# brown-ivl/manus

Measured on AMD Instinct MI355X. Metric: train iters/sec (fwd+bwd) 300k Gaussians @1080p, 8 views; PSNR parity, higher is better.
Workload: dtype f32

## Files before the change

include/manus_hip.h:

```cpp
#ifndef MANUS_HIP_H
#define MANUS_HIP_H

#include <stddef.h>
#include <stdint.h>

#ifdef __cplusplus
extern "C" {
#endif

#define MGR_VERSION 100
#define MGR_CAM_FLOATS 40
#define MGR_TILE 16
#define MGR_MAX_BONES 32

enum {
    MGR_OK = 0,
    MGR_EINVAL = -1,
    MGR_ENOMEM = -2,
    MGR_EHIP = -3,
    MGR_EOVERFLOW = -4,
    MGR_ECUT = -6,
    MGR_ETIER = -7
};

// ... 30 lines not shown
                       const float* xyz, const float* log_scale, const float* rot,
                       const float* opacity_logit, const float* f_dc, const float* f_rest,
                       const float* skin_w, const float* transforms, const int32_t* radii,
                       const float* out_color, const float* dL_dcolor, float grad2d_scale, float* d_xyz,
                       float* d_log_scale, float* d_rot, float* d_opacity_logit, float* d_f_dc,
                       float* d_f_rest, float* d_skin_w, float* stat_grad2d, float* stat_vis,
                       int32_t* stat_radii, void* workspace, size_t workspace_bytes,
                       int64_t pair_capacity, int debug, void* stream);



int mgr_views_active_list(void* workspace, int V, int N, int W, int H, int64_t pair_capacity, const uint32_t** list,
                          const uint32_t** count);

int mgr_views_backward_run_lists(int on);

int mgr_sh_to_half(int N, const float* f_rest, void* out_half, void* stream);

int mgr_raster_layout(int V, int N, int W, int H, int64_t pair_capacity, size_t* out, int n_out);
int mgr_raster_record_bytes(void);

int mgr_raster_set_cut_margin(float frac_entries, int min_entries, float depth_range_frac, float depth_rel, int interior_only);
int mgr_raster_set_cut_penalty(int forwards);
int mgr_raster_set_status_mirror(const void* workspace, void* host_words);
int mgr_raster_status_tiers_sync(const void* workspace, int64_t* num_pairs, int32_t* overflow, int32_t* tiers,
                                 void* stream);
int mgr_raster_status_sync(const void* workspace, int64_t* num_pairs, int32_t* overflow,
                           void* stream);

int mgr_raster_debug_binning_sync(const void* workspace, int V, int N, int W, int H,
// ... 150 lines not shown
```

manus_amd/_lib.py:

```python
import ctypes
import os

import weakref

import torch

_HERE = os.path.dirname(os.path.abspath(__file__))
_VARIANT = os.environ.get("MANUS_HIP_VARIANT", "")
LIB_PATH = os.path.join(_HERE, "libmanus_hip%s.so" % ("_" + _VARIANT if _VARIANT else ""))
_LIB = None

MGR_CAM_FLOATS = 40
MGR_MAX_BONES = 32

c_int, c_i64, c_f32, c_vp, c_sz = ctypes.c_int, ctypes.c_int64, ctypes.c_float, ctypes.c_void_p, ctypes.c_size_t

SIGNATURES = {
    "mgr_version": (c_int, []),
    "mgr_build_variant": (c_int, []),
    "mgr_raster_repair_max_tiles": (c_int, []),
    "mgr_last_error": (ctypes.c_char_p, []),
    "mgr_raster_workspace_bytes": (c_sz, [c_int, c_int, c_int, c_int, c_i64]),
    "mgr_raster_forward": (c_int, [c_int, c_int, c_int, c_int, c_vp, c_vp, c_vp, c_i64, c_vp, c_i64, c_vp,
                                   c_i64, c_vp, c_i64, c_vp, c_vp, c_vp, c_sz, c_i64, c_int, c_vp]),
# ... 9 lines not shown
    "mgr_raster_set_status_mirror": (c_int, [c_vp, c_vp]),
    "mgr_raster_set_cut_margin": (c_int, [c_f32, c_int, c_f32, c_f32, c_int]),
    "mgr_raster_set_cut_penalty": (c_int, [c_int]),
    "mgr_raster_status_tiers_sync": (c_int, [c_vp, ctypes.POINTER(c_i64), ctypes.POINTER(ctypes.c_int32),
                                             ctypes.POINTER(ctypes.c_int32), c_vp]),
    "mgr_debug_pair_alpha": (c_int, [c_int, c_vp, c_vp, c_vp, c_vp, c_vp, c_vp]),
    "mgr_raster_debug_binning_sync": (c_int, [c_vp, c_int, c_int, c_int, c_int, c_i64, c_int, c_vp, c_vp,
                                              c_i64, c_vp]),
    "mgr_skin_weights_fwd": (c_int, [c_int, c_vp, c_vp, c_int, c_int, c_int, c_int, c_int, c_vp, c_vp, c_vp,
                                     c_vp]),
    "mgr_skin_weights_bwd": (c_int, [c_int, c_vp, c_vp, c_int, c_int, c_int, c_int, c_int, c_vp, c_vp, c_vp,
                                     c_vp, c_int, c_vp]),
    "mgr_skin_weights_bwd_indexed": (c_int, [c_int, c_vp, c_vp, c_int, c_int, c_int, c_int, c_int, c_vp, c_vp, c_vp,
                                             c_vp, c_vp, c_vp, c_int, c_vp]),
    "mgr_views_backward_run_lists": (c_int, [c_int]),
    "mgr_views_active_list": (c_int, [c_vp, c_int, c_int, c_int, c_int, c_i64, ctypes.POINTER(c_vp), ctypes.POINTER(c_vp)]),
    "mgr_lbs_cov_fwd": (c_int, [c_int, c_int, c_int, c_vp, c_vp, c_vp, c_vp, c_vp, c_vp, c_vp, c_vp, c_vp]),
    "mgr_lbs_cov_bwd": (c_int, [c_int, c_int, c_int, c_vp, c_vp, c_vp, c_vp, c_vp, c_vp, c_vp, c_vp, c_vp,
                                c_vp, c_vp, c_vp, c_vp]),
    "mgr_lbs_cov_fwd_rows": (c_int, [c_int, c_int, c_int, c_vp, c_vp, c_vp, c_vp, c_vp, c_vp, c_vp, c_vp, c_int, c_vp]),
    "mgr_lbs_cov_bwd_rows": (c_int, [c_int, c_int, c_int, c_vp, c_vp, c_vp, c_vp, c_vp, c_vp, c_vp, c_vp, c_int, c_vp,
                                     c_vp, c_vp, c_vp, c_vp]),
    "mgr_sh_color_fwd_rows": (c_int, [c_int, c_int, c_vp, c_vp, c_i64, c_vp, c_i64, c_int, c_vp, c_vp, c_vp]),
    "mgr_sh_color_bwd_rows": (c_int, [c_int, c_int, c_vp, c_vp, c_i64, c_vp, c_i64, c_int, c_vp, c_vp, c_vp, c_vp, c_vp,
                                      c_vp]),
    "mgr_sh_color_fwd": (c_int, [c_int, c_int, c_vp, c_vp, c_i64, c_vp, c_i64, c_vp, c_vp, c_vp]),
    "mgr_sh_color_bwd": (c_int, [c_int, c_int, c_vp, c_vp, c_i64, c_vp, c_i64, c_vp, c_vp, c_vp, c_vp, c_vp,
                                 c_vp]),
    "mgr_pack_camera": (c_int, [c_f32, c_f32, c_vp, c_vp, c_vp, c_vp, c_vp]),
    "mgr_bone_transforms": (c_int, [c_int, c_int, c_vp, c_vp, c_vp, c_vp]),
# ... 172 lines not shown
```

manus_amd/csrc/mgr_common.h:

```cpp
#pragma once
#include <hip/hip_runtime.h>
#include <stdint.h>
#include <stdio.h>
#include <string.h>

#include "../../include/manus_hip.h"

#define MGR_WAVE 64

extern thread_local char g_mgr_err[512];

static inline int mgr_fail(int code, const char* fmt, const char* a = "", const char* b = "") {
    snprintf(g_mgr_err, sizeof(g_mgr_err), fmt, a, b);
    return code;
}

#define MGR_HIP(call)                                                                      \
    do {                                                                                   \
        hipError_t e_ = (call);                                                            \
        if (e_ != hipSuccess) return mgr_fail(MGR_EHIP, "%s: %s", #call, hipGetErrorString(e_)); \
    } while (0)

#define MGR_LAUNCH_CHECK(name, stream, debug)                                              \
    do {                                                                                   \
// ... 106 lines not shown
    int32_t pad;
#if MGR_GREC_BYTES == 64
    int32_t pad64[4];
#endif
};

#define MGR_CHUNK 64

static inline uint32_t mgr_rep_units(int64_t cap) { int64_t u = cap / 16384; return (uint32_t)(u < 64 ? 64 : (u > 1024 ? 1024 : u)); }
static inline uint32_t mgr_rep_list(int64_t cap) { int64_t n = cap / 8; return (uint32_t)(n < (1 << 16) ? (1 << 16) : (n > (2 << 20) ? (2 << 20) : n)); }
static inline uint32_t mgr_rep_ck(int64_t cap) { return mgr_rep_list(cap) / MGR_CHUNK + mgr_rep_units(cap); }

struct MgrLayout {
    size_t header, scan_part, scan_cls, scan_box, grec, depth, rect, alive, pair_off, tile_count, tile_start, tile_cursor, tile_done, tile_qdone,
        tile_zcut, tile_zused, tile_qend, tile_bgok, tile_queue, tile_qrec, chunk_start, items, ckpt, keys, keys2, groups, sorted_gid, final_T, n_contrib, pair_tag, pair_grad, inst_grad, inst_tag,
        db_count, db_cursor, db_start, db_nvis, db_bbox, db_keys, db_order, db_rec, bin_mat, tile_rep, rep_unit, rep_state, rep_last, rep_cnt, rep_cand, rep_view, tile_zwin, db_zrange, db_item, total;
};

#ifndef MGR_DB_BUCKETS
#define MGR_DB_BUCKETS 1024
#endif
#ifndef MGR_DB_ITEM
#define MGR_DB_ITEM 768
#endif
#define MGR_DB_RANK_MAX 2048
#define MGR_DB_RANK_LARGE 3072
#ifndef MGR_BIN_BLOCK
#define MGR_BIN_BLOCK 1024
#endif
static inline int mgr_bin_block(int V, int N) { return (long long)V * (long long)N >= 500000ll ? MGR_BIN_BLOCK : 256; }

static inline size_t mgr_align(size_t x) { return (x + 255) & ~(size_t)255; }

static inline MgrLayout mgr_layout(int V, int N, int W, int H, int64_t cap) {
    MgrLayout L;
    size_t VN = (size_t)V * (size_t)(N > 0 ? N : 1);
    size_t gx = (W + MGR_TILE - 1) / MGR_TILE, gy = (H + MGR_TILE - 1) / MGR_TILE;
    size_t VT = (size_t)V * gx * gy, VP = (size_t)V * W * H;
    size_t c = (size_t)(cap > 0 ? cap : 1);
    size_t o = 0;
    L.header = o;      o += mgr_align(sizeof(MgrHeader));
    const size_t scan_blocks = (size_t)V * ((gx * gy + 1023) / 1024);
    L.scan_part = o;   o += mgr_align((scan_blocks + 1) * 8);
    L.scan_cls = o;    o += mgr_align(scan_blocks * 34 * 4);
    L.scan_box = o;    o += mgr_align(scan_blocks * 16);
    L.grec = o;        o += mgr_align(VN * sizeof(MgrGRec));
    L.depth = o;       o += mgr_align(VN * 4);
    L.rect = o;        o += mgr_align(VN * 8);
// ... 34 lines not shown
        L.db_order = o;  o += mgr_align(VN * 4);
        L.db_rec = o;    o += mgr_align(VN * 16);
        L.bin_mat = o;   o += mgr_align((size_t)V * nblk * gx * gy * 4);
    }
    L.tile_bgok = o; o += mgr_align((size_t)V * gx * gy);
    L.tile_rep = o;  o += mgr_align(VT * 4);
    L.rep_unit = o;  o += mgr_align(rep_u * sizeof(MgrRepUnit));
    L.rep_state = o; o += mgr_align(rep_u * 64 * 16);
    L.rep_last = o;  o += mgr_align(rep_u * 64 * 4);
    L.rep_cnt = o;   o += mgr_align(rep_u * 4);
    L.rep_cand = o;  o += mgr_align(rep_u * (size_t)MGR_REP_CAND * 8);
    L.rep_view = o;  o += mgr_align((size_t)V * sizeof(MgrRepView));
    L.tile_zwin = o; o += mgr_align(VT * 4);
    L.db_zrange = o; o += mgr_align((size_t)V * (((size_t)(N > 0 ? N : 1) + 511) / 512) * 2 * 4);
    L.db_item = o;   o += mgr_align((size_t)V * (((size_t)(N > 0 ? N : 1) + MGR_DB_ITEM - 1) / MGR_DB_ITEM + 1) * 2 * 4);
    L.total = o;
    return L;
}

#ifdef __HIPCC__

struct MgrCam {
    float tanfovx, tanfovy;
    float view[16], proj[16];
    float campos[3];
};

__device__ __forceinline__ void mgr_load_cam(const float* __restrict__ cams, int v, MgrCam& c) {
    const float* p = cams + (size_t)v * MGR_CAM_FLOATS;
    c.tanfovx = p[0];
    c.tanfovy = p[1];
#pragma unroll
    for (int i = 0; i < 16; ++i) {
        c.view[i] = p[2 + i];
// ... 305 lines not shown
```

manus_amd/csrc/raster_bwd.hip:

```cpp
#include <atomic>

#include "instance_math.h"

#ifdef MGR_STATS
__device__ unsigned long long g_stats[16];
extern "C" int mgr_debug_stats(unsigned long long* dst) {
    return (int)hipMemcpyFromSymbol(dst, HIP_SYMBOL(g_stats), sizeof(unsigned long long) * 16);
}
__device__ unsigned long long g_bhist[3][65];
extern "C" int mgr_debug_bhist(unsigned long long* dst) {
    return (int)hipMemcpyFromSymbol(dst, HIP_SYMBOL(g_bhist), sizeof(unsigned long long) * 3 * 65);
}
#define BH(r, c, v) do { const int c_ = (c); const unsigned long long v_ = (unsigned long long)(v); if (lane == 0) atomicAdd(&g_bhist[r][c_], v_); } while (0)
#define MGR_STAT(i, v) do { const unsigned long long v_ = (unsigned long long)(v); if (lane == 0) atomicAdd(&g_stats[i], v_); } while (0)
#else
#define MGR_STAT(i, v)
#endif

#ifdef BWD_PROF
__device__ unsigned long long g_bprof[8];
extern "C" int mgr_debug_bprof(unsigned long long* dst) {
    return (int)hipMemcpyFromSymbol(dst, HIP_SYMBOL(g_bprof), sizeof(unsigned long long) * 8);
}
#define BP(k) { const long long now_ = wall_clock64(); acc_[k] += now_ - tp_; tp_ = now_; }
// ... 26 lines not shown
    return bits;
}
#define MGR_LDS_VOLATILE_F32 volatile const __attribute__((address_space(3))) float*
#define BWD_ROW 288
#define BWD_PLANE_W 64
#define BWD_PLANE_B 128
#ifndef BWD_WAVES
#define BWD_WAVES 4
#endif

__global__ __launch_bounds__(256) __attribute__((amdgpu_waves_per_eu(BWD_WAVES, BWD_WAVES))) void k_blend_bwd(
    int N, int W, int H, int gx, int gy, const uint32_t* __restrict__ sorted_gid, const MgrGRec* __restrict__ grec,
    const uint32_t* __restrict__ n_contrib, const float4* __restrict__ ckpt, const uint4* __restrict__ items,
    MgrHeader* hdr, const float* __restrict__ out_color, const float* __restrict__ dL_dpix,
    uint32_t* __restrict__ pair_tag, float4* __restrict__ pair_grad, uint32_t* __restrict__ inst_tag, uint32_t cap,
    uint32_t epoch) {
    __shared__ __align__(16) float s_pair[4][32][MGR_PAIR_FLOATS];
    __shared__ __align__(16) float s_xch[4][4 * BWD_ROW];
    __shared__ float s_acc[4][BWD_BATCH][9];
    __shared__ uint32_t s_flag[4][BWD_BATCH];

    const int tid = threadIdx.x, wave = tid >> 6, lane = tid & 63;
    const int T = gx * gy;
    const uint32_t n_items = hdr->n_items;
    if (blockIdx.x == 0 && tid < 4) (tid == 3 ? hdr->n_active : hdr->n_runs[tid]) = 0;
    if (blockIdx.x == 0 && tid == 4) hdr->bwd_seq += 1u;
    const size_t P = (size_t)W * H;
    const unsigned long long lt = (1ull << lane) - 1ull;
    float* const slab = &s_pair[wave][0][0];
    float* const xch = &s_xch[wave][0];
    float* const acc = &s_acc[wave][0][0];
    uint32_t* const flag = &s_flag[wave][0];
    const int e2 = lane >> 3, pc = lane & 7;
#ifdef BWD_PROF
    long long acc_[6] = {0, 0, 0, 0, 0, 0}, tp_ = wall_clock64(), nit_ = 0;
#endif

    MgrQueue queue;
    queue.init(hdr->qctr, n_items, (int)blockIdx.x);
    uint32_t item = queue.resolve(queue.issue(lane), lane);
    while (item != 0xFFFFFFFFu) {
        const uint32_t next_raw = queue.issue(lane);
        const uint4 recA = items[2 * (size_t)item], recB = items[2 * (size_t)item + 1];
        const uint32_t vt = recA.x, chunk = recA.y;
        const uint32_t mxq[4] = {recB.x, recB.y, recB.z, recB.w};
        const int v = (int)(vt / (uint32_t)T), t = (int)(vt % (uint32_t)T);
        const int bx = t % gx, by = t / gx;
        const uint32_t first = chunk * BWD_BATCH;
        const uint32_t tmax = max(max(mxq[0], mxq[1]), max(mxq[2], mxq[3]));
        const int cnt = (int)min((uint32_t)BWD_BATCH, tmax - first);
        const MgrGRec* const gv = grec + (size_t)v * N;
#ifdef BWD_PROF
        ++nit_;
#endif
        BP(0);
#if BWD_KO & 1024
        const uint32_t gid = sorted_gid[recA.z] + 0u * (uint32_t)lane;
#else
        const uint32_t gid = sorted_gid[recA.z + (uint32_t)min(lane, cnt - 1)];
// ... 1 lines not shown
        float4 ra, rb, rcz;
        {
            const MgrGRec* r = gv + gid;
            ra = *(const float4*)r;
            rb = *((const float4*)r + 1);
            rcz = *((const float4*)r + 2);
        }
#pragma unroll
        for (int k = 0; k < 9; ++k) acc[k * 64 + lane] = 0.f;
        flag[lane] = 0u;
        const int32_t slot = __float_as_int(rcz.y) + by * __float_as_int(rcz.z) + bx;
        const float qmax_e = mgr_qmax(rb.y);
        BP(1);

        uint32_t qmask = (mxq[0] > first ? 1u : 0u) | (mxq[1] > first ? 2u : 0u) | (mxq[2] > first ? 4u : 0u) | (mxq[3] > first ? 8u : 0u);
        struct PxState {
            uint32_t nc;
            float t0, t1, t2, o0, o1, o2;
            float4 ck;
        };
        auto load_px = [&](int quad, PxState& q) {
            const int px = bx * 16 + (quad & 1) * 8 + (lane & 7);
            const int py = by * 16 + (quad >> 1) * 8 + (lane >> 3);
            const size_t pixc = (size_t)min(py, H - 1) * W + min(px, W - 1);
#if BWD_KO & 512
            q.nc = tmax; q.t0 = 0.001f * (float)pixc; q.t1 = 0.5f; q.t2 = 0.25f; q.o0 = 0.3f; q.o1 = 0.2f; q.o2 = 0.1f;
            q.ck = make_float4(0.1f, 0.1f, 0.1f, 0.5f);
#else
            q.nc = n_contrib[(size_t)v * P + pixc];
            const float* gp = dL_dpix + (size_t)v * 3 * P + pixc;
// ... 44 lines not shown
                xch[xoff] = g0; xch[64 + xoff] = g1; xch[128 + xoff] = g2;
                __builtin_amdgcn_wave_barrier();
#pragma unroll
                for (int j = 0; j < 2; ++j) {
                    const float4 a4 = *(const float4*)(xch + 4 * pc + 32 * j), b4 = *(const float4*)(xch + 64 + 4 * pc + 32 * j),
                                 c4 = *(const float4*)(xch + 128 + 4 * pc + 32 * j);
                    gr0[2 * j] = mgr_v2f{a4.x, a4.y}; gr0[2 * j + 1] = mgr_v2f{a4.z, a4.w};
                    gr1[2 * j] = mgr_v2f{b4.x, b4.y}; gr1[2 * j + 1] = mgr_v2f{b4.z, b4.w};
                    gr2[2 * j] = mgr_v2f{c4.x, c4.y}; gr2[2 * j + 1] = mgr_v2f{c4.z, c4.w};
                }
                __builtin_amdgcn_wave_barrier();
            }
            const float fx_col = qx0 + (float)pc;
            const mgr_v2f g0v = {g0, g0}, g1v = {g1, g1}, g2v = {g2, g2};
            bool alive = false;
            if (lane < cnt && first + (uint32_t)lane < wlast)
                alive = !mgr_box_dead(ra.x, ra.y, ra.z, ra.w, rb.x, qmax_e, qx0 + (float)bx0, qy0 + (float)by0,
                                      qx0 + (float)bx1, qy0 + (float)by1);
            const unsigned long long m = __ballot(alive);
            const int na = __popcll(m);
            MGR_STAT(0, __popcll(__ballot(lane < cnt)));
            MGR_STAT(1, na);
            if (alive) {
                const int rank = __popcll(m & lt);
                float* pb = slab + (rank >> 1) * MGR_PAIR_FLOATS;
                mgr_pair_store(pb, rank & 1, ra.x, ra.y, ra.z, ra.w, rb.x, rb.y, rb.z, rb.w, rcz.x,
                               first + (uint32_t)lane + 1u);
                if ((na & 1) && rank == na - 1) mgr_pair_pad(pb);
            }
            const int npair = (BWD_KO & 4) ? ((na + 1) >> 1) * 57 / 100 : (na + 1) >> 1;
#ifdef MGR_STATS
            MGR_STAT(8, (unsigned long long)npair * __popcll(__ballot(last > first)));
            MGR_STAT(9, npair);
// ... 767 lines not shown
    }
    const int b8 = (n8 + IB_THREADS / 8 - 1) / (IB_THREADS / 8), b4 = (n4 + IB_THREADS / 4 - 1) / (IB_THREADS / 4);
    if constexpr (NVV >= 8) {
        if (blk < b8) { inst_bwd_body<8, BMAX, MIXED, SH_HALF, true, NVV>(blk, n8, active_list, MGR_IB_ARGS); return; }
    }
    blk -= b8;
    if constexpr (NVV >= 4) {
        if (blk < b4) { inst_bwd_body<4, BMAX, MIXED, SH_HALF, true, NVV>(blk, n4, active_list + (size_t)N, MGR_IB_ARGS); return; }
    }
    blk -= b4;
    inst_bwd_body<2, BMAX, MIXED, SH_HALF, true, NVV>(blk, n2, active_list + 2 * (size_t)N, MGR_IB_ARGS);
}

static std::atomic<int> g_inst_runs{[] { const char* e = getenv("MANUS_INST_RUNS"); return e ? atoi(e) : 1; }()};
extern "C" int mgr_views_backward_run_lists(int on) { return g_inst_runs.exchange(on); }

struct CanonGrads {
    int B, n_art, sh_half;
    const float *xyz, *log_scale, *rot, *op_logit, *f_dc, *f_rest, *skin_w, *transforms;
    const int32_t* radii;
    float grad2d_scale;
    float *d_xyz, *d_ls, *d_rot, *d_op, *d_fdc, *d_frest, *d_w, *st_grad2d, *st_vis;
    int32_t* st_radii;
};

static int raster_backward_impl(int V, int N, int W, int H, const float* cams, const float* bg,
                                   const float* means3D, int64_t s_means, const float* cov3D,
                                   int64_t s_cov, const float* colors, int64_t s_col,
                                   const float* opacity, int64_t s_op, const float* out_color,
                                   const float* dL_dcolor, float* dL_dmeans3D, float* dL_dmeans2D, float* dL_dcolors,
// ... 9 lines not shown
    if (!canon && (!means3D || !cov3D || !dL_dmeans3D || !dL_dmeans2D || !dL_dcolors || !dL_dopacity || !dL_dcov3D))
        return mgr_fail(MGR_EINVAL, "mgr_raster_backward: null pointer");
    const int gx = (W + 15) / 16, gy = (H + 15) / 16;
    const MgrLayout L = mgr_layout(V, N, W, H, cap);
    if (workspace_bytes < L.total) return mgr_fail(MGR_ENOMEM, "mgr_raster_backward: workspace too small");
    char* ws = (char*)workspace;
    MgrHeader* hdr = (MgrHeader*)(ws + L.header);
    static std::atomic<uint32_t> g_epoch{0};
    uint32_t epoch = g_epoch.fetch_add(1) + 1;
    if (epoch == 0) epoch = g_epoch.fetch_add(1) + 1;

    { MGR_PROF("k_blend_bwd", stream); hipLaunchKernelGGL(k_blend_bwd, dim3(256 * BWD_WAVES), dim3(256), 0, stream, N, W, H, gx, gy,
                       (const uint32_t*)(ws + L.sorted_gid), (const MgrGRec*)(ws + L.grec), (const uint32_t*)(ws + L.n_contrib),
                       (const float4*)(ws + L.ckpt), (const uint4*)(ws + L.items), hdr, out_color,
                       dL_dcolor, (uint32_t*)(ws + L.pair_tag), (float4*)(ws + L.pair_grad),
                       (uint32_t*)(ws + L.inst_tag), (uint32_t)cap, epoch); }
    MGR_LAUNCH_CHECK("k_blend_bwd", stream, debug & 1);
    if (canon) {
        const int Gv = V <= 1 ? 1 : V <= 2 ? 2 : V <= 4 ? 4 : 8;
        const int ipb = 256 / Gv;
        const size_t lds = (size_t)Gv * (MGR_CAM_FLOATS + (canon->skin_w ? IB_TSTRIDE(canon->B) : 0)) * sizeof(float);
        float4* iacc = (float4*)(ws + L.inst_grad);
        uint32_t* alist = (uint32_t*)(ws + L.inst_grad + (size_t)N * Gv * 48);
        const int ipb2 = IB_THREADS / Gv;
        const bool mixed = canon->skin_w && canon->n_art < N;
        int rounds = (int)((long long)N / ((long long)ipb * 1024));
        rounds = rounds < 1 ? 1 : (rounds > IG_ROUNDS ? IG_ROUNDS : rounds);
        const dim3 grid((N + ipb2 - 1) / ipb2), grid_g((N + ipb * rounds - 1) / (ipb * rounds));
        for (int v0 = 0; v0 < V; v0 += Gv) {
            const int vc = V - v0 < Gv ? V - v0 : Gv;
            const int accm = v0 > 0 ? 1 : 0;
// ... 138 lines not shown
```

manus_amd/csrc/raster_fwd.hip:

```cpp
#include <atomic>
#include <mutex>

#include "instance_math.h"
#include "il_list.h"

#include <cstdlib>
#include <cstring>
#include <map>
#include <string>
#include <vector>

thread_local char g_mgr_err[512] = {0};

int g_mgr_prof_on = 0;
namespace {
struct ProfRec { const char* name; hipEvent_t a, b; };
std::vector<ProfRec> g_prof_recs;
std::vector<hipEvent_t> g_prof_pool;
hipEvent_t prof_event() {
    if (!g_prof_pool.empty()) { hipEvent_t e = g_prof_pool.back(); g_prof_pool.pop_back(); return e; }
    hipEvent_t e;
    if (hipEventCreate(&e) != hipSuccess) return nullptr;
    return e;
}
// ... 1838 lines not shown
    return (int)e;
}
#endif
__device__ __forceinline__ float mgr_sel(unsigned long long m, float a, float b) {
    float r;
    asm("v_cndmask_b32 %0, %1, %2, %3" : "=v"(r) : "v"(b), "v"(a), "s"(m));
    return r;
}
__device__ __forceinline__ uint32_t mgr_selu(unsigned long long m, uint32_t a, uint32_t b) {
    uint32_t r;
    asm("v_cndmask_b32 %0, %1, %2, %3" : "=v"(r) : "v"(b), "v"(a), "s"(m));
    return r;
}
__device__ __forceinline__ bool mgr_fwd_pair_step(const float4& R0, const float4& R1, const float4& R2, const float4& R3, const float4& R4,
                                                  const mgr_v2f fpx2, const mgr_v2f fpy2, float& Tr, mgr_v2f& C01, float& C2, uint32_t& last,
                                                  unsigned long long& done_m, const unsigned long long exec_m) {
    mgr_v2f al;
    unsigned long long ma, mb;
    mgr_pair_alpha_masks(R0, R1, R2, fpx2, fpy2, al, ma, mb);
    {
        const unsigned long long keep = ma & ~done_m;
        const float a = mgr_sel(keep, al.x, 0.0f);
        const float testT = Tr * (1.0f - a);
        const unsigned long long stop = __builtin_amdgcn_ballot_w64(testT < 0.0001f);
        const unsigned long long contrib = keep & ~stop;
        const float w = mgr_sel(contrib, a * Tr, 0.0f);
        C01 += mgr_v2f{R3.x, R3.y} * w;
        C2 += R4.x * w;
        Tr = mgr_sel(stop, Tr, testT);
        last = mgr_selu(contrib, __float_as_uint(R4.z), last);
        done_m |= stop;
    }
    {
        const unsigned long long keep = mb & ~done_m;
        const float a = mgr_sel(keep, al.y, 0.0f);
        const float testT = Tr * (1.0f - a);
        const unsigned long long stop = __builtin_amdgcn_ballot_w64(testT < 0.0001f);
        const unsigned long long contrib = keep & ~stop;
        const float w = mgr_sel(contrib, a * Tr, 0.0f);
        C01 += mgr_v2f{R3.z, R3.w} * w;
        C2 += R4.y * w;
        Tr = mgr_sel(stop, Tr, testT);
        last = mgr_selu(contrib, __float_as_uint(R4.w), last);
        done_m |= stop;
    }
    return (~done_m & exec_m) == 0ull;
}
#define FWD_SLOTS 64
__global__ __launch_bounds__(256) FWD_OCC void k_blend_fwd(int N, int W, int H, int gx, int gy, int VT,
                                                     const float* __restrict__ bg,
                                                     const uint32_t* __restrict__ tile_queue,
                                                     const uint4* __restrict__ tile_qrec,
                                                     const uint32_t* __restrict__ sorted_gid,
                                                     const MgrGRec* __restrict__ grec,
                                                     float* __restrict__ out_color,
                                                     uint32_t* __restrict__ n_contrib,
                                                     uint32_t* __restrict__ tile_done,
                                                     uint32_t* __restrict__ tile_qdone,
                                                     float4* __restrict__ ckpt, MgrHeader* hdr,
                                                     const uint32_t* __restrict__ tile_zused, uint32_t* __restrict__ tile_qend, int skip_fill) {
    __shared__ __align__(16) float s_pair[4][32][MGR_PAIR_FLOATS];
    __shared__ __align__(16) uint4 s_qrec[FWD_SLOTS];
    __shared__ uint32_t s_step[FWD_SLOTS];
    __shared__ uint32_t s_claim;
    const int tid = threadIdx.x, lane = tid & 63;
    const int wave = __builtin_amdgcn_readfirstlane(tid >> 6);
    const int T = gx * gy;
    const uint32_t n_busy = hdr->queue_len;
    const uint32_t n_queue = hdr->queue_len_i;
    const size_t P = (size_t)W * H;
    const float bg0 = bg[0], bg1 = bg[1], bg2 = bg[2];
    const unsigned long long lt = (1ull << lane) - 1ull;
    float* const slab = &s_pair[wave][0][0];
    const uint32_t gid_max = (uint32_t)(N > 0 ? N - 1 : 0);

// ... 166 lines not shown
                const uint32_t nxt = queue.resolve(raw, lane);
                uint4 nrec = make_uint4(END, 0u, 0u, 0u);
                if (nxt != END) nrec = tile_qrec[nxt];
#ifdef FWD_KO_DEEP
                if (nxt != END && nxt < FWD_KO_DEEP) nrec.x = MGR_HOLE;
#endif
                if (lane == 0) {
                    s_qrec[(step + 1u) % FWD_SLOTS] = nrec;
                    __builtin_amdgcn_fence(__ATOMIC_RELEASE, "workgroup");
                    __hip_atomic_store(&s_step[(step + 1u) % FWD_SLOTS], step + 1u, __ATOMIC_RELAXED, __HIP_MEMORY_SCOPE_WORKGROUP);
                }
                provided = true;
            }
            const int npair = (cnt + 1) >> 1;
            FP(1);
            auto pair_step = [&](const float4& R0, const float4& R1, const float4& R2, const float4& R3, const float4& R4) -> bool {
                return mgr_fwd_pair_step(R0, R1, R2, R3, R4, fpx2, fpy2, Tr, C01, C2, last, done_m, exec_m);
            };
#ifdef FWD_LDS_PIPE1
            for (int p = 0; p < npair; ++p) {
                const float4* pp = (const float4*)(slab + p * MGR_PAIR_FLOATS);
                const float4 R0 = pp[0], R1 = pp[1], R2 = pp[2], R3 = pp[3], R4 = pp[4];
                if (pair_step(R0, R1, R2, R3, R4)) break;
            }
#else
            if (npair > 0) {
                const float4* pa = (const float4*)slab;
                float4 A0 = pa[0], A1 = pa[1], A2 = pa[2];
                for (int p = 0;; p += 2) {
                    const float4* pb = (const float4*)(slab + min(p + 1, 31) * MGR_PAIR_FLOATS);
                    const float4 B0 = pb[0], B1 = pb[1], B2 = pb[2];
                    const float4* pc = (const float4*)(slab + p * MGR_PAIR_FLOATS);
                    const float4 A3 = pc[3], A4 = pc[4];
                    __builtin_amdgcn_sched_barrier(0);
                    if (pair_step(A0, A1, A2, A3, A4) || p + 1 >= npair) break;
                    const float4* pn = (const float4*)(slab + min(p + 2, 31) * MGR_PAIR_FLOATS);
                    A0 = pn[0]; A1 = pn[1]; A2 = pn[2];
                    const float4 B3 = pb[3], B4 = pb[4];
                    __builtin_amdgcn_sched_barrier(0);
                    if (pair_step(B0, B1, B2, B3, B4) || p + 2 >= npair) break;
                }
            }
#endif
            FP(2);
            const uint32_t nextpos = off + 64u;
            if ((nextpos % MGR_CHUNK) == 0 && nextpos < nlist && (((~done_m & exec_m) >> lane) & 1ull))
                ckpt[(size_t)(ck0 + nextpos / MGR_CHUNK - 1) * 256 + pslot] = make_float4(C01.x, C01.y, C2, Tr);
#ifndef FWD_PF1
            rec = rec1;
            rec1 = rec2;
#endif
            FP(3);
        }
        FP(3);
        if (!provided) {
            const uint32_t nxt = queue.resolve(raw, lane);
            uint4 nrec = make_uint4(END, 0u, 0u, 0u);
            if (nxt != END) nrec = tile_qrec[nxt];
#ifdef FWD_KO_DEEP
            if (nxt != END && nxt < FWD_KO_DEEP) nrec.x = MGR_HOLE;
#endif
            if (lane == 0) {
// ... 296 lines not shown
                                      qy0 + (float)by1);
            }
            const unsigned long long m = __ballot(alive);
            const int cnt = __popcll(m);
            if (alive) {
                const int rank = __popcll(m & lt);
                float* pb = slab + (rank >> 1) * MGR_PAIR_FLOATS;
                mgr_pair_store<true>(pb, rank & 1, r.x, r.y, r.ca, r.cb, r.cc, r.op, r.r, r.g, r.b, nl + j + (uint32_t)lane + 1u);
                if ((cnt & 1) && rank == cnt - 1) mgr_pair_pad<true>(pb);
            }
            __builtin_amdgcn_wave_barrier();
            const int npair = (cnt + 1) >> 1;
            for (int p = 0; p < npair; ++p) {
                const float4* pp = (const float4*)(slab + p * MGR_PAIR_FLOATS);
                const float4 R0 = pp[0], R1 = pp[1], R2 = pp[2], R3 = pp[3], R4 = pp[4];
                if (mgr_fwd_pair_step(R0, R1, R2, R3, R4, fpx2, fpy2, Tr, C01, C2, last, done_m, exec_m)) break;
            }
            __builtin_amdgcn_wave_barrier();
            const uint32_t nextpos = nl + j + blen;
            if ((nextpos % MGR_CHUNK) == 0u && nextpos < total && (((~done_m & exec_m) >> lane) & 1ull))
                ckpt[(size_t)(ov_ck0 + nextpos / MGR_CHUNK - c0) * 256 + pslot] = make_float4(C01.x, C01.y, C2, Tr);
            j += blen;
        }
        if (inside) {
            const size_t pix = (size_t)py * W + px;
            n_contrib[(size_t)v * P + pix] = last;
            float* o = out_color + (size_t)v * 3 * P + pix;
            o[0] = C01.x + Tr * bg0;
            o[P] = C01.y + Tr * bg1;
            o[2 * P] = C2 + Tr * bg2;
        }
// ... 124 lines not shown
    const uint32_t base = s_base;
    for (uint32_t i = (uint32_t)tid; i < total; i += 256u) {
        int lo = 0, hi = 256;
        while (hi - lo > 1) {
            const int mid = (lo + hi) >> 1;
            if (s_run[mid] <= i) lo = mid; else hi = mid;
        }
        const uint32_t c = i - s_run[lo];
        const uint4 r = s_qr[lo], x = s_rp[lo];
        uint32_t off = r.y + c * MGR_CHUNK, ck = r.w + (c > 0 ? c - 1 : 0);
        const uint32_t p0 = x.x & 0x7FFFFFFFu;
        if (x.x != 0u && c * MGR_CHUNK >= p0) {
            off = x.y + (c * MGR_CHUNK - p0);
            ck = c * MGR_CHUNK == p0 ? x.w : x.z + (c - p0 / MGR_CHUNK);
        }
        items[2 * (size_t)(base + i)] = make_uint4(r.x, c, off, ck);
        items[2 * (size_t)(base + i) + 1] = s_qd[lo];
    }
}

struct CanonInputs {
    int B, n_art, sh_half;
    const float *xyz, *log_scale, *rot, *op_logit, *f_dc, *f_rest, *skin_w, *transforms;
};

struct MgrSideStream {
    hipStream_t stream = nullptr;
    hipEvent_t fork = nullptr, join = nullptr;
    hipError_t init() {
        if (stream) return hipSuccess;
        hipError_t e = hipStreamCreateWithFlags(&stream, hipStreamNonBlocking);
// ... 268 lines not shown
                           (const unsigned long long*)(ws + L.keys), (uint32_t*)(ws + L.sorted_gid), hdr,
                           (uint32_t)cap); }
        MGR_HIP(hipEventRecord(side.join, side.stream));
        { MGR_PROF("k_tile_sort", stream); hipLaunchKernelGGL(k_tile_sort, dim3(512), dim3(RS_THREADS), SORT_LDS_KEYS * 8 + RS_WAVES * 256 * 4 + 256, stream,
                           tile_start, (const uint32_t*)(ws + L.tile_queue),
                           (const unsigned long long*)(ws + L.keys), (const unsigned long long*)(ws + L.keys2),
                           (const uint4*)(ws + L.groups), (uint32_t*)(ws + L.sorted_gid), hdr, (uint32_t)cap); }
        MGR_HIP(hipStreamWaitEvent(stream, side.join, 0));
        MGR_LAUNCH_CHECK("k_tile_sort", stream, debug);
    }
    }
    if (!do_blend) return MGR_OK;
    { MGR_PROF("k_blend_fwd", stream); hipLaunchKernelGGL(k_blend_fwd, dim3(MGR_FWD_GRID), dim3(256), 0, stream, N, W, H, gx, gy, VT, bg,
                       (const uint32_t*)(ws + L.tile_queue), (const uint4*)(ws + L.tile_qrec), (const uint32_t*)(ws + L.sorted_gid), (const MgrGRec*)(ws + L.grec), out_color,
                       (uint32_t*)(ws + L.n_contrib), (uint32_t*)(ws + L.tile_done), (uint32_t*)(ws + L.tile_qdone),
                       (float4*)(ws + L.ckpt), hdr, (const uint32_t*)(ws + L.tile_zused), (uint32_t*)(ws + L.tile_qend), bg_filled ? 1 : 0); }
    if (repair && N > 0) {
        { MGR_PROF("k_repair_scan", stream);
          hipLaunchKernelGGL(k_repair_prep, dim3(V), dim3(256), 0, stream, T, gx, hdr, rep_all, (const uint32_t*)(ws + L.tile_zused),
                             (const uint32_t*)(ws + L.tile_zwin));
          hipLaunchKernelGGL(k_repair_scan, dim3(REP_SCAN_SEGS, V), dim3(REP_SCAN_THREADS), 0, stream, N, T, gx, hdr, rep_all, (const int32_t*)radii,
                             (const ushort4*)(ws + L.rect), (const float*)(ws + L.depth), (const MgrGRec*)(ws + L.grec)); }
        { MGR_PROF("k_repair_blend", stream);
          hipLaunchKernelGGL(k_repair_blend, dim3(128), dim3(RS_THREADS), REP_BLEND_LDS, stream, N, W, H, gx, T, hdr, rep_all, bg,
                             (uint32_t*)(ws + L.sorted_gid), (const MgrGRec*)(ws + L.grec), out_color, (uint32_t*)(ws + L.n_contrib),
                             (uint32_t*)(ws + L.tile_qdone), (float4*)(ws + L.ckpt)); }
        MGR_LAUNCH_CHECK("k_repair_blend", stream, debug);
    }
    IlListArgs ll = mgr_take_loss_list(workspace);
    if (ll.nbx) {
        if (ll.H != H || ll.W != W || ll.list_views != V) return mgr_fail(MGR_EINVAL, "attached loss list: views or image size differ from the forward's");
// ... 36 lines not shown
    return raster_forward_impl(V, N, W, H, cams, bg, nullptr, 0, nullptr, 0, nullptr, 0, nullptr, 0, &ci, out_color,
                               radii, workspace, workspace_bytes, cap, debug, stream_);
}

#ifdef BIN_PROF
extern "C" int mgr_binprof(unsigned long long* out) {
    MGR_HIP(hipMemcpyFromSymbol(out, HIP_SYMBOL(g_binprof), 8 * 8 * 4096));
    return 0;
}
#endif
extern "C" int mgr_raster_layout(int V, int N, int W, int H, int64_t cap, size_t* out, int n_out) {
    const MgrLayout L = mgr_layout(V, N, W, H, cap);
    const size_t v[] = {L.header, L.grec, L.depth, L.rect, L.alive, L.pair_off, L.tile_count, L.tile_start,
                        L.tile_cursor, L.tile_done, L.tile_queue, L.chunk_start, L.items, L.ckpt, L.keys,
                        L.sorted_gid, L.final_T, L.n_contrib, L.pair_tag, L.pair_grad, L.total, L.inst_grad, L.inst_tag,
                        L.db_nvis, L.db_bbox, L.db_order, L.tile_zcut, L.tile_zused, L.tile_qend, L.tile_rep, L.rep_unit, L.rep_cnt, L.tile_zwin};
    const int n = (int)(sizeof(v) / sizeof(v[0]));
    for (int i = 0; i < n && i < n_out; ++i) out[i] = v[i];
    return n;
}

__global__ void k_debug_pair_alpha(int n, const float* __restrict__ rec, const int32_t* __restrict__ px,
                                   const int32_t* __restrict__ py, float* __restrict__ alpha, int32_t* __restrict__ valid) {
    const int i = blockIdx.x * blockDim.x + threadIdx.x;
    if (i >= n) return;
    float pb[MGR_PAIR_FLOATS];
    const float* r = rec + (size_t)i * 6;
    mgr_pair_store(pb, 0, r[0], r[1], r[2], r[3], r[4], r[5], 0.f, 0.f, 0.f, 1u);
    mgr_pair_pad(pb);
    const float4 R0 = make_float4(pb[0], pb[1], pb[2], pb[3]), R1 = make_float4(pb[4], pb[5], pb[6], pb[7]),
                 R2 = make_float4(pb[8], pb[9], pb[10], pb[11]);
// ... 80 lines not shown
```

Baseline: 771.4.

## Record per-chunk contributor masks in forward blend and reuse them in backward

The forward blend kernel now records, for each 64-entry chunk and pixel quad, a ballot mask of the Gaussians that actually contributed. The backward blend reads these masks instead of re-running the conservative box-dead test, and drops quads with no contributors. This cuts wasted per-Gaussian work in the backward pass, at the cost of an extra workspace buffer and extra forward stores. Items from repair/other paths are flagged with the top bit of the chunk field so they fall back to the box test.

```diff
diff --git a/include/manus_hip.h b/include/manus_hip.h
--- a/include/manus_hip.h
+++ b/include/manus_hip.h
@@ -68,6 +68,8 @@
                           const uint32_t** count);
 
 int mgr_views_backward_run_lists(int on);
+
+int mgr_raster_bwd_boxtest(int on);
 
 int mgr_sh_to_half(int N, const float* f_rest, void* out_half, void* stream);
 
diff --git a/manus_amd/_lib.py b/manus_amd/_lib.py
--- a/manus_amd/_lib.py
+++ b/manus_amd/_lib.py
@@ -47,6 +47,7 @@
     "mgr_skin_weights_bwd_indexed": (c_int, [c_int, c_vp, c_vp, c_int, c_int, c_int, c_int, c_int, c_vp, c_vp, c_vp,
                                              c_vp, c_vp, c_vp, c_int, c_vp]),
     "mgr_views_backward_run_lists": (c_int, [c_int]),
+    "mgr_raster_bwd_boxtest": (c_int, [c_int]),
     "mgr_views_active_list": (c_int, [c_vp, c_int, c_int, c_int, c_int, c_i64, ctypes.POINTER(c_vp), ctypes.POINTER(c_vp)]),
     "mgr_lbs_cov_fwd": (c_int, [c_int, c_int, c_int, c_vp, c_vp, c_vp, c_vp, c_vp, c_vp, c_vp, c_vp, c_vp]),
     "mgr_lbs_cov_bwd": (c_int, [c_int, c_int, c_int, c_vp, c_vp, c_vp, c_vp, c_vp, c_vp, c_vp, c_vp, c_vp,
diff --git a/manus_amd/csrc/mgr_common.h b/manus_amd/csrc/mgr_common.h
--- a/manus_amd/csrc/mgr_common.h
+++ b/manus_amd/csrc/mgr_common.h
@@ -144,7 +144,7 @@
 struct MgrLayout {
     size_t header, scan_part, scan_cls, scan_box, grec, depth, rect, alive, pair_off, tile_count, tile_start, tile_cursor, tile_done, tile_qdone,
         tile_zcut, tile_zused, tile_qend, tile_bgok, tile_queue, tile_qrec, chunk_start, items, ckpt, keys, keys2, groups, sorted_gid, final_T, n_contrib, pair_tag, pair_grad, inst_grad, inst_tag,
-        db_count, db_cursor, db_start, db_nvis, db_bbox, db_keys, db_order, db_rec, bin_mat, tile_rep, rep_unit, rep_state, rep_last, rep_cnt, rep_cand, rep_view, tile_zwin, db_zrange, db_item, total;
+        db_count, db_cursor, db_start, db_nvis, db_bbox, db_keys, db_order, db_rec, bin_mat, tile_rep, rep_unit, rep_state, rep_last, rep_cnt, rep_cand, rep_view, tile_zwin, db_zrange, db_item, cmask, total;
 };
 
 #ifndef MGR_DB_BUCKETS
@@ -162,6 +162,9 @@
 
 static inline size_t mgr_align(size_t x) { return (x + 255) & ~(size_t)255; }
 
+static inline size_t mgr_cmask_nck(int64_t cap) {
+    return (size_t)(cap > 0 ? cap : 1) / MGR_CHUNK + 1 + mgr_rep_ck(cap);
+}
 static inline MgrLayout mgr_layout(int V, int N, int W, int H, int64_t cap) {
     MgrLayout L;
     size_t VN = (size_t)V * (size_t)(N > 0 ? N : 1);
@@ -226,10 +229,14 @@
     L.tile_zwin = o; o += mgr_align(VT * 4);
     L.db_zrange = o; o += mgr_align((size_t)V * (((size_t)(N > 0 ? N : 1) + 511) / 512) * 2 * 4);
     L.db_item = o;   o += mgr_align((size_t)V * (((size_t)(N > 0 ? N : 1) + MGR_DB_ITEM - 1) / MGR_DB_ITEM + 1) * 2 * 4);
+    L.cmask = o;     o += mgr_align((mgr_cmask_nck(cap) + VT) * 4 * 8);
     L.total = o;
     return L;
 }
 
+__host__ __device__ __forceinline__ size_t mgr_cmask_word(uint32_t vt, uint32_t chunk, uint32_t ck, uint32_t quad, size_t nck) {
+    return (chunk ? (size_t)ck : nck + vt) * 4 + quad;
+}
 #ifdef __HIPCC__
 
 struct MgrCam {
diff --git a/manus_amd/csrc/raster_bwd.hip b/manus_amd/csrc/raster_bwd.hip
--- a/manus_amd/csrc/raster_bwd.hip
+++ b/manus_amd/csrc/raster_bwd.hip
@@ -64,7 +64,7 @@
     const uint32_t* __restrict__ n_contrib, const float4* __restrict__ ckpt, const uint4* __restrict__ items,
     MgrHeader* hdr, const float* __restrict__ out_color, const float* __restrict__ dL_dpix,
     uint32_t* __restrict__ pair_tag, float4* __restrict__ pair_grad, uint32_t* __restrict__ inst_tag, uint32_t cap,
-    uint32_t epoch) {
+    uint32_t epoch, const unsigned long long* __restrict__ cmask, size_t nck) {
     __shared__ __align__(16) float s_pair[4][32][MGR_PAIR_FLOATS];
     __shared__ __align__(16) float s_xch[4][4 * BWD_ROW];
     __shared__ float s_acc[4][BWD_BATCH][9];
@@ -92,7 +92,7 @@
     while (item != 0xFFFFFFFFu) {
         const uint32_t next_raw = queue.issue(lane);
         const uint4 recA = items[2 * (size_t)item], recB = items[2 * (size_t)item + 1];
-        const uint32_t vt = recA.x, chunk = recA.y;
+        const uint32_t vt = recA.x, chunk = recA.y & 0x7FFFFFFFu;
         const uint32_t mxq[4] = {recB.x, recB.y, recB.z, recB.w};
         const int v = (int)(vt / (uint32_t)T), t = (int)(vt % (uint32_t)T);
         const int bx = t % gx, by = t / gx;
@@ -124,6 +124,13 @@
         BP(1);
 
         uint32_t qmask = (mxq[0] > first ? 1u : 0u) | (mxq[1] > first ? 2u : 0u) | (mxq[2] > first ? 4u : 0u) | (mxq[3] > first ? 8u : 0u);
+        const bool use_cm = cmask != nullptr && (recA.y >> 31) == 0u;
+        unsigned long long cmw[4] = {~0ull, ~0ull, ~0ull, ~0ull};
+        if (use_cm) {
+#pragma unroll
+            for (int q = 0; q < 4; ++q) cmw[q] = cmask[mgr_cmask_word(vt, chunk, recA.w, (uint32_t)q, nck)];
+            qmask &= (cmw[0] ? 1u : 0u) | (cmw[1] ? 2u : 0u) | (cmw[2] ? 4u : 0u) | (cmw[3] ? 8u : 0u);
+        }
         struct PxState {
             uint32_t nc;
             float t0, t1, t2, o0, o1, o2;
@@ -198,9 +205,15 @@
             const float fx_col = qx0 + (float)pc;
             const mgr_v2f g0v = {g0, g0}, g1v = {g1, g1}, g2v = {g2, g2};
             bool alive = false;
-            if (lane < cnt && first + (uint32_t)lane < wlast)
-                alive = !mgr_box_dead(ra.x, ra.y, ra.z, ra.w, rb.x, qmax_e, qx0 + (float)bx0, qy0 + (float)by0,
-                                      qx0 + (float)bx1, qy0 + (float)by1);
+            if (lane < cnt && first + (uint32_t)lane < wlast) {
+                if (use_cm) {
+                    const unsigned long long cmq = quad == 0 ? cmw[0] : quad == 1 ? cmw[1] : quad == 2 ? cmw[2] : cmw[3];
+                    alive = (cmq >> lane) & 1ull;
+                } else {
+                    alive = !mgr_box_dead(ra.x, ra.y, ra.z, ra.w, rb.x, qmax_e, qx0 + (float)bx0, qy0 + (float)by0,
+                                          qx0 + (float)bx1, qy0 + (float)by1);
+                }
+            }
             const unsigned long long m = __ballot(alive);
             const int na = __popcll(m);
             MGR_STAT(0, __popcll(__ballot(lane < cnt)));
@@ -998,6 +1011,8 @@
 
 static std::atomic<int> g_inst_runs{[] { const char* e = getenv("MANUS_INST_RUNS"); return e ? atoi(e) : 1; }()};
 extern "C" int mgr_views_backward_run_lists(int on) { return g_inst_runs.exchange(on); }
+static std::atomic<int> g_bwd_boxtest{0};
+extern "C" int mgr_raster_bwd_boxtest(int on) { return g_bwd_boxtest.exchange(on); }
 
 struct CanonGrads {
     int B, n_art, sh_half;
@@ -1037,7 +1052,8 @@
                        (const uint32_t*)(ws + L.sorted_gid), (const MgrGRec*)(ws + L.grec), (const uint32_t*)(ws + L.n_contrib),
                        (const float4*)(ws + L.ckpt), (const uint4*)(ws + L.items), hdr, out_color,
                        dL_dcolor, (uint32_t*)(ws + L.pair_tag), (float4*)(ws + L.pair_grad),
-                       (uint32_t*)(ws + L.inst_tag), (uint32_t)cap, epoch); }
+                       (uint32_t*)(ws + L.inst_tag), (uint32_t)cap, epoch,
+                       g_bwd_boxtest ? (const unsigned long long*)nullptr : (const unsigned long long*)(ws + L.cmask), mgr_cmask_nck(cap)); }
     MGR_LAUNCH_CHECK("k_blend_bwd", stream, debug & 1);
     if (canon) {
         const int Gv = V <= 1 ? 1 : V <= 2 ? 2 : V <= 4 ? 4 : 8;
diff --git a/manus_amd/csrc/raster_fwd.hip b/manus_amd/csrc/raster_fwd.hip
--- a/manus_amd/csrc/raster_fwd.hip
+++ b/manus_amd/csrc/raster_fwd.hip
@@ -1876,7 +1876,7 @@
 }
 __device__ __forceinline__ bool mgr_fwd_pair_step(const float4& R0, const float4& R1, const float4& R2, const float4& R3, const float4& R4,
                                                   const mgr_v2f fpx2, const mgr_v2f fpy2, float& Tr, mgr_v2f& C01, float& C2, uint32_t& last,
-                                                  unsigned long long& done_m, const unsigned long long exec_m) {
+                                                  unsigned long long& done_m, const unsigned long long exec_m, uint32_t& cb) {
     mgr_v2f al;
     unsigned long long ma, mb;
     mgr_pair_alpha_masks(R0, R1, R2, fpx2, fpy2, al, ma, mb);
@@ -1892,6 +1892,7 @@
         Tr = mgr_sel(stop, Tr, testT);
         last = mgr_selu(contrib, __float_as_uint(R4.z), last);
         done_m |= stop;
+        cb = contrib != 0ull ? 1u : 0u;
     }
     {
         const unsigned long long keep = mb & ~done_m;
@@ -1905,6 +1906,7 @@
         Tr = mgr_sel(stop, Tr, testT);
         last = mgr_selu(contrib, __float_as_uint(R4.w), last);
         done_m |= stop;
+        cb |= contrib != 0ull ? 2u : 0u;
     }
     return (~done_m & exec_m) == 0ull;
 }
@@ -1920,7 +1922,8 @@
                                                      uint32_t* __restrict__ tile_done,
                                                      uint32_t* __restrict__ tile_qdone,
                                                      float4* __restrict__ ckpt, MgrHeader* hdr,
-                                                     const uint32_t* __restrict__ tile_zused, uint32_t* __restrict__ tile_qend, int skip_fill) {
+                                                     const uint32_t* __restrict__ tile_zused, uint32_t* __restrict__ tile_qend, int skip_fill,
+                                                     unsigned long long* __restrict__ cmask, size_t nck) {
     __shared__ __align__(16) float s_pair[4][32][MGR_PAIR_FLOATS];
     __shared__ __align__(16) uint4 s_qrec[FWD_SLOTS];
     __shared__ uint32_t s_step[FWD_SLOTS];
@@ -2117,14 +2120,18 @@
             }
             const int npair = (cnt + 1) >> 1;
             FP(1);
-            auto pair_step = [&](const float4& R0, const float4& R1, const float4& R2, const float4& R3, const float4& R4) -> bool {
-                return mgr_fwd_pair_step(R0, R1, R2, R3, R4, fpx2, fpy2, Tr, C01, C2, last, done_m, exec_m);
+            unsigned long long cm = 0ull;
+            auto pair_step = [&](int p, const float4& R0, const float4& R1, const float4& R2, const float4& R3, const float4& R4) -> bool {
+                uint32_t cb;
+                const bool end = mgr_fwd_pair_step(R0, R1, R2, R3, R4, fpx2, fpy2, Tr, C01, C2, last, done_m, exec_m, cb);
+                cm |= (unsigned long long)cb << (2 * p);
+                return end;
             };
 #ifdef FWD_LDS_PIPE1
             for (int p = 0; p < npair; ++p) {
                 const float4* pp = (const float4*)(slab + p * MGR_PAIR_FLOATS);
                 const float4 R0 = pp[0], R1 = pp[1], R2 = pp[2], R3 = pp[3], R4 = pp[4];
-                if (pair_step(R0, R1, R2, R3, R4)) break;
+                if (pair_step(p, R0, R1, R2, R3, R4)) break;
             }
 #else
             if (npair > 0) {
@@ -2136,12 +2143,12 @@
                     const float4* pc = (const float4*)(slab + p * MGR_PAIR_FLOATS);
                     const float4 A3 = pc[3], A4 = pc[4];
                     __builtin_amdgcn_sched_barrier(0);
-                    if (pair_step(A0, A1, A2, A3, A4) || p + 1 >= npair) break;
+                    if (pair_step(p, A0, A1, A2, A3, A4) || p + 1 >= npair) break;
                     const float4* pn = (const float4*)(slab + min(p + 2, 31) * MGR_PAIR_FLOATS);
                     A0 = pn[0]; A1 = pn[1]; A2 = pn[2];
                     const float4 B3 = pb[3], B4 = pb[4];
                     __builtin_amdgcn_sched_barrier(0);
-                    if (pair_step(B0, B1, B2, B3, B4) || p + 2 >= npair) break;
+                    if (pair_step(p + 1, B0, B1, B2, B3, B4) || p + 2 >= npair) break;
                 }
             }
 #endif
@@ -2149,6 +2156,10 @@
             const uint32_t nextpos = off + 64u;
             if ((nextpos % MGR_CHUNK) == 0 && nextpos < nlist && (((~done_m & exec_m) >> lane) & 1ull))
                 ckpt[(size_t)(ck0 + nextpos / MGR_CHUNK - 1) * 256 + pslot] = make_float4(C01.x, C01.y, C2, Tr);
+            {
+                const unsigned long long pm = __builtin_amdgcn_ballot_w64(((m >> lane) & 1ull) && ((cm >> __popcll(m & lt)) & 1ull));
+                if (lane == 0) cmask[mgr_cmask_word(vt, off / MGR_CHUNK, ck0 + off / MGR_CHUNK - 1u, quad, nck)] = pm;
+            }
 #ifndef FWD_PF1
             rec = rec1;
             rec1 = rec2;
@@ -2475,7 +2486,8 @@
             for (int p = 0; p < npair; ++p) {
                 const float4* pp = (const float4*)(slab + p * MGR_PAIR_FLOATS);
                 const float4 R0 = pp[0], R1 = pp[1], R2 = pp[2], R3 = pp[3], R4 = pp[4];
-                if (mgr_fwd_pair_step(R0, R1, R2, R3, R4, fpx2, fpy2, Tr, C01, C2, last, done_m, exec_m)) break;
+                uint32_t cb_;
+                if (mgr_fwd_pair_step(R0, R1, R2, R3, R4, fpx2, fpy2, Tr, C01, C2, last, done_m, exec_m, cb_)) break;
             }
             __builtin_amdgcn_wave_barrier();
             const uint32_t nextpos = nl + j + blen;
@@ -2630,7 +2642,7 @@
             off = x.y + (c * MGR_CHUNK - p0);
             ck = c * MGR_CHUNK == p0 ? x.w : x.z + (c - p0 / MGR_CHUNK);
         }
-        items[2 * (size_t)(base + i)] = make_uint4(r.x, c, off, ck);
+        items[2 * (size_t)(base + i)] = make_uint4(r.x, c | (x.x != 0u ? 0x80000000u : 0u), off, ck);
         items[2 * (size_t)(base + i) + 1] = s_qd[lo];
     }
 }
@@ -2929,7 +2941,8 @@
     { MGR_PROF("k_blend_fwd", stream); hipLaunchKernelGGL(k_blend_fwd, dim3(MGR_FWD_GRID), dim3(256), 0, stream, N, W, H, gx, gy, VT, bg,
                        (const uint32_t*)(ws + L.tile_queue), (const uint4*)(ws + L.tile_qrec), (const uint32_t*)(ws + L.sorted_gid), (const MgrGRec*)(ws + L.grec), out_color,
                        (uint32_t*)(ws + L.n_contrib), (uint32_t*)(ws + L.tile_done), (uint32_t*)(ws + L.tile_qdone),
-                       (float4*)(ws + L.ckpt), hdr, (const uint32_t*)(ws + L.tile_zused), (uint32_t*)(ws + L.tile_qend), bg_filled ? 1 : 0); }
+                       (float4*)(ws + L.ckpt), hdr, (const uint32_t*)(ws + L.tile_zused), (uint32_t*)(ws + L.tile_qend), bg_filled ? 1 : 0,
+                       (unsigned long long*)(ws + L.cmask), mgr_cmask_nck(cap)); }
     if (repair && N > 0) {
         { MGR_PROF("k_repair_scan", stream);
           hipLaunchKernelGGL(k_repair_prep, dim3(V), dim3(256), 0, stream, T, gx, hdr, rep_all, (const uint32_t*)(ws + L.tile_zused),
@@ -2996,7 +3009,7 @@
     const size_t v[] = {L.header, L.grec, L.depth, L.rect, L.alive, L.pair_off, L.tile_count, L.tile_start,
                         L.tile_cursor, L.tile_done, L.tile_queue, L.chunk_start, L.items, L.ckpt, L.keys,
                         L.sorted_gid, L.final_T, L.n_contrib, L.pair_tag, L.pair_grad, L.total, L.inst_grad, L.inst_tag,
-                        L.db_nvis, L.db_bbox, L.db_order, L.tile_zcut, L.tile_zused, L.tile_qend, L.tile_rep, L.rep_unit, L.rep_cnt, L.tile_zwin};
+                        L.db_nvis, L.db_bbox, L.db_order, L.tile_zcut, L.tile_zused, L.tile_qend, L.tile_rep, L.rep_unit, L.rep_cnt, L.tile_zwin, L.cmask};
     const int n = (int)(sizeof(v) / sizeof(v[0]));
     for (int i = 0; i < n && i < n_out; ++i) out[i] = v[i];
     return n;
```

New measurement: 758.4, median of 2. 1.7% lower.
